# amzn/pecos

Measured on NVIDIA H100. Metric: XR-Linear top-10 queries/sec, higher is better.
Workload: dtype f32

## Files before the change

### include/pecos_b200.h

```cpp
#ifndef PECOS_B200_H_
#define PECOS_B200_H_

#include <stdbool.h>
#include <stddef.h>
#include <stdint.h>

#ifdef __cplusplus
extern "C" {
#endif

typedef struct {
    uint32_t rows, cols;
    uint64_t* col_ptr;
    uint32_t* row_idx;
    float* val;
} ScipyCscF32;

typedef struct {
    uint32_t rows, cols;
    uint64_t* row_ptr;
    uint32_t* col_idx;
    float* val;
} ScipyCsrF32;

// ... 166 lines not shown
void pb200_hnsw_launch_info(void* model_ptr, uint64_t* out);
void pb200_hnsw_get_info(void* model_ptr, uint64_t* out);
int pb200_hnsw_host_info(const char* model_dir, int metric, int sparse, uint64_t* out);
uint32_t pb200_hnsw_vcap_retries(void* model_ptr);



void pb200_sparse_block_distances(int device, int metric, const void* row_ptr, const void* ent, const void* q_ids, uint32_t nq,
                                  const void* col_ptr, const void* post, uint32_t c0, uint32_t nc, void* out, void* work,
                                  void* stream);
void pb200_sparse_candidate_distances(int device, int metric, const void* row_ptr, const void* ent, const void* cand, uint32_t n,
                                      uint32_t C, void* out, void* work, void* stream);

void* pb200_xlinear_host_load(const char* model_path, int kind);
void* pb200_xlinear_host_from_csc(const ScipyCscF32* W, const ScipyCscF32* C, float bias);
void* pb200_xlinear_host_prefix_layer(void* hptr);
void pb200_xlinear_host_free(void* hptr);
uint32_t pb200_xlinear_host_depth(void* hptr);
void pb200_xlinear_host_layer_dims(void* hptr, uint32_t layer, uint64_t* out);
void pb200_xlinear_host_layer_export(void* hptr, uint32_t layer, void* chunks32, uint32_t* meta, void* entries8,
                                     uint32_t* label_of_col);
int pb200_xlinear_host_plan_fits(void* hptr, uint32_t beam_size, uint32_t only_topk, uint32_t* out);
int pb200_xlinear_plan_fits(void* ptr, uint32_t beam_size, uint32_t only_topk, uint32_t* out);
uint32_t pb200_xlinear_plan_stride(void* ptr, int host, uint32_t beam_size, uint32_t only_topk);
uint32_t pb200_xlinear_beam_limit(int topk);

#ifdef __cplusplus
}
#endif
#endif
```

### pecos_b200/core.py

```python
import ctypes
import os
from ctypes import (
    CFUNCTYPE,
    POINTER,
    byref,
    c_bool,
    c_char_p,
    c_double,
    c_float,
    c_int,
    c_int32,
    c_size_t,
    c_uint32,
    c_uint64,
    c_void_p,
    cast,
)

import numpy as np
import scipy.sparse as smat

LIB_BASENAME = "libpecos_b200_float32.so"
LIB_DIR = os.path.join(os.path.dirname(os.path.abspath(__file__)), "lib")
LIB_PATH = os.path.join(LIB_DIR, LIB_BASENAME)
# ... 412 lines not shown
        fp(c.pb200_hnsw_get_counters, None, [c_void_p, POINTER(c_uint64)])
        fp(c.pb200_hnsw_set_stages, c_int, [c_void_p, c_int])
        fp(c.pb200_hnsw_launch_info, None, [c_void_p, POINTER(c_uint64)])
        fp(c.pb200_hnsw_get_info, None, [c_void_p, POINTER(c_uint64)])
        fp(c.pb200_hnsw_host_info, c_int, [c_char_p, c_int, c_int, POINTER(c_uint64)])
        fp(c.pb200_pairwise_ann_get_counters, None, [c_void_p, POINTER(c_uint64)])
        fp(c.pb200_pairwise_ann_kernel_ms, c_double, [c_void_p])
        fp(c.pb200_pairwise_ann_launch_info, None, [c_void_p, POINTER(c_uint64)])
        fp(c.pb200_pairwise_ann_dense_fits, c_int, [c_uint32, POINTER(c_uint32)])
        fp(c.pb200_pairwise_ann_host_info, c_int, [c_char_p, c_int, POINTER(c_uint64)])
        fp(c.pb200_sparse_block_distances, None, [c_int, c_int, c_void_p, c_void_p, c_void_p, c_uint32, c_void_p, c_void_p,
                                                  c_uint32, c_uint32, c_void_p, c_void_p, c_void_p])
        fp(c.pb200_sparse_candidate_distances, None, [c_int, c_int, c_void_p, c_void_p, c_void_p, c_uint32, c_uint32, c_void_p,
                                                      c_void_p, c_void_p])
        fp(c.pb200_xlinear_host_load, c_void_p, [c_char_p, c_int])
        fp(c.pb200_xlinear_host_prefix_layer, c_void_p, [c_void_p])
        fp(c.pb200_xlinear_host_free, None, [c_void_p])
        fp(c.pb200_xlinear_host_depth, c_uint32, [c_void_p])
        fp(c.pb200_xlinear_host_layer_dims, None, [c_void_p, c_uint32, POINTER(c_uint64)])
        fp(c.pb200_xlinear_host_layer_export, None, [c_void_p, c_uint32, c_void_p, c_void_p, c_void_p, c_void_p])
        fp(c.pb200_xlinear_host_plan_fits, c_int, [c_void_p, c_uint32, c_uint32, POINTER(c_uint32)])
        fp(c.pb200_xlinear_plan_fits, c_int, [c_void_p, c_uint32, c_uint32, POINTER(c_uint32)])
        fp(c.pb200_xlinear_plan_stride, c_uint32, [c_void_p, c_int, c_uint32, c_uint32])
        fp(c.pb200_xlinear_beam_limit, c_uint32, [c_int])
        fp(c.pb200_xlinear_cm_info, c_int, [c_void_p, c_int, POINTER(c_uint64)])

    def xlinear_check_layer_beam(self, b_prev):
        limit = int(self.clib_float32.pb200_xlinear_beam_limit(1))
        if b_prev > limit:
            raise ValueError(f"pecos_b200: the beam entering this layer would hold {b_prev} nodes, more than the supported "
                             f"maximum of {limit}")
# ... 30 lines not shown
        owner = _PinnedOwner(self, ptr, buf)
        arr = np.frombuffer(owner.buf, dtype=dtype, count=int(n))
        return _PinnedArray(arr, owner)

    def host_layer_layout_from_csc(self, W, C, bias):
        cw = ScipyCscF32.init_from(smat.csc_matrix(W, dtype=np.float32))
        cc = ScipyCscF32.init_from(smat.csc_matrix(C, dtype=np.float32))
        h = c_void_p(self.clib_float32.pb200_xlinear_host_from_csc(byref(cw), byref(cc), c_float(bias)))
        return self._export_host_model(h)

    def host_model_layout(self, model_path, is_mmap=False):
        c = self.clib_float32
        h = c_void_p(c.pb200_xlinear_host_load(model_path.encode("utf-8"), 1 if is_mmap else 0))
        return self._export_host_model(h)

    def host_prefix_layer_layout(self, model_path):
        c = self.clib_float32
        h = c_void_p(c.pb200_xlinear_host_load(model_path.encode("utf-8"), 0))
        try:
            m = c_void_p(c.pb200_xlinear_host_prefix_layer(h))
        finally:
            c.pb200_xlinear_host_free(h)
        return self._export_host_model(m)[0]

    def _export_host_model(self, h):
        c = self.clib_float32
        try:
            layers = []
            for d in range(c.pb200_xlinear_host_depth(h)):
                dims = (c_uint64 * 8)()
                c.pb200_xlinear_host_layer_dims(h, d, dims)
                w_rows, n_cols, out_cols, n_chunks, c_max, meta_len, n_ent, n_lab = [int(x) for x in dims]
                chunks = np.zeros(n_chunks, dtype=CHUNK_HEADER_DTYPE)
                meta = np.zeros(meta_len, dtype=np.uint32)
                entries = np.zeros(n_ent, dtype=CHUNK_ENTRY_DTYPE)
# ... 42 lines not shown
```

### pecos_b200/csrc/c_api.cu

```cuda
#include "../../include/pecos_b200.h"

#include <algorithm>
#include <atomic>
#include <cstdio>
#include <cstdlib>
#include <cstring>
#include <memory>
#include <exception>
#include <mutex>
#include <string>
#include <thread>
#include <unordered_set>
#include <vector>

#include "hnsw_build_sparse.h"
#include "hnsw_engine.h"
#include "pairwise_engine.h"
#include "xlinear_engine.h"

namespace {

std::atomic<int> g_device{0};

[[noreturn]] void die(const char* where, const char* what) {
// ... 693 lines not shown
    std::unique_ptr<pb200::XLinearHostModel> m =
        kind == 1 ? pb200::load_xlinear_mmap_model(model_path, false)
                  : pb200::load_xlinear_npz_model(model_path, pb200::LT_BINARY_SEARCH_CHUNKED);
    return m.release();
    PB200_API_END("pb200_xlinear_host_load")
}

void* pb200_xlinear_host_from_csc(const ScipyCscF32* W, const ScipyCscF32* C, float bias) {
    PB200_API_BEGIN
    const pb200::CscRaw w{W->rows, W->cols, W->col_ptr, W->row_idx, W->val};
    const pb200::CscRaw c{C->rows, C->cols, C->col_ptr, C->row_idx, C->val};
    return pb200::make_single_layer_model(w, c, bias).release();
    PB200_API_END("pb200_xlinear_host_from_csc")
}

void* pb200_xlinear_host_prefix_layer(void* hptr) {
    PB200_API_BEGIN
    const auto& H = *static_cast<pb200::XLinearHostModel*>(hptr);
    if (H.depth() < 2) throw std::runtime_error("pecos_b200: the prefix layer needs a model of depth >= 2");
    auto m = std::make_unique<pb200::XLinearHostModel>();
    m->layers.resize(1);
    pb200::build_prefix_layer(H.layers[0], H.layers[1], m->layers[0]);
    return m.release();
    PB200_API_END("pb200_xlinear_host_prefix_layer")
}

void pb200_xlinear_host_free(void* hptr) { delete static_cast<pb200::XLinearHostModel*>(hptr); }

int pb200_xlinear_host_plan_fits(void* hptr, uint32_t beam_size, uint32_t only_topk, uint32_t* out) {
    PB200_API_BEGIN
    if (!hptr) throw std::runtime_error("null host model");
    return plan_fits(*static_cast<pb200::XLinearHostModel*>(hptr), beam_size, only_topk, out);
    PB200_API_END("pb200_xlinear_host_plan_fits")
}

int pb200_xlinear_plan_fits(void* ptr, uint32_t beam_size, uint32_t only_topk, uint32_t* out) {
    PB200_API_BEGIN
    return plan_fits(xlinear_of(ptr).primary().host(), beam_size, only_topk, out);
    PB200_API_END("pb200_xlinear_plan_fits")
}
// ... 458 lines not shown
```

### pecos_b200/csrc/xlinear_cm_kernel.cuh

```cuda
#pragma once

constexpr int kCmFeat = 8;
constexpr int kCmSlots = 4;
constexpr int kCmMaxWarps = 16;
constexpr int kCmMinWarps = 4;
constexpr uint32_t kCmMaxDup = 400;
constexpr uint32_t kCmSmemBudget = 224u << 10;
constexpr uint32_t kCmMinReuse = 24;
constexpr uint32_t kCmMinPairsPerSm = 48u;
constexpr uint32_t kCmDirectRows = 16384;
constexpr uint32_t kCmEmpty = 0xFFFFFFFFu;

struct CmWork {
    uint32_t* slot_pos;
    uint32_t* count;
    uint32_t* bucket_ptr;
    uint64_t* cost_ptr;
    uint32_t* pair_q;
    uint32_t* pair_pos;
    uint32_t* claim;
    uint32_t* active;
};

struct CmPlan {
    bool eligible = false;
    uint32_t warps = 0, grid = 0;
    size_t smem = 0;
};

constexpr uint32_t kCmPrefixTop0 = 8;
struct CmPrefixOut {
    uint32_t rows = 0;
    uint32_t n0 = 0;
    int pp_kind = 0, pp_p = 0;
    const ChunkHeader* chunks1 = nullptr;
    uint32_t* beam_id = nullptr;
    float* beam_val = nullptr;
    uint32_t* beam_cnt = nullptr;
    uint32_t beam_stride = 0;
    float* cand1 = nullptr;
    uint64_t cand1_stride = 0;
};

__host__ __device__ inline uint32_t cm_align16(uint32_t x) { return (x + 15u) & ~15u; }

__host__ __device__ constexpr uint32_t cm_buffers(uint32_t stages) { return stages + 1u; }

__host__ __device__ inline size_t cm_warp_bytes(uint32_t acc_cols, uint32_t stages) {
// ... 332 lines not shown
}

__device__ inline uint32_t cm_start_chunk(const CmWork& w, uint32_t n_vc, uint32_t b, uint32_t shares) {
    const uint64_t T = w.cost_ptr[n_vc];
    if (T == 0) return n_vc;
    const uint64_t t = static_cast<uint64_t>(T / shares) * b + (T % shares) * b / shares;
    uint32_t lo = 0, hi = n_vc;
    while (hi - lo > 1) {
        const uint32_t mid = (lo + hi) >> 1;
        if (w.cost_ptr[mid] <= t) lo = mid; else hi = mid;
    }
    return lo;
}

enum { kCmPhSwitch, kCmPhCopy, kCmPhStaging, kCmPhLookup, kCmPhAccumulate, kCmPhSlice, kCmPhases };
#ifdef PB200_CM_TRACE
constexpr uint32_t kCmTraceCtas = 1024;
constexpr uint32_t kCmTraceWarp = kCmPhases + 4;
constexpr uint32_t kCmTraceCta = 3 + kCmMaxWarps * kCmTraceWarp;
__device__ unsigned long long g_cm_trace[3 + kCmTraceCtas * kCmTraceCta];
__device__ __forceinline__ unsigned long long cm_globaltimer() {
    unsigned long long t;
    asm volatile("mov.u64 %0, %%globaltimer;" : "=l"(t));
    return t;
}
struct CmTrace {
    unsigned long long start;
    long long t, ph[kCmPhases];
    unsigned long long trips, slots;
    unsigned long long slices, pairs, images;
// ... 62 lines not shown
    const unsigned short* __restrict__ rp_s = reinterpret_cast<const unsigned short*>(img + S.off_rp);
    const float* __restrict__ ew_s = reinterpret_cast<const float*>(img + S.off_ew);
    const unsigned char* __restrict__ ec_s = img + S.off_ec;
    const int lane = threadIdx.x & 31;
    const int warp = threadIdx.x >> 5;
    const int nwarps = blockDim.x >> 5;
    constexpr int kStride = kCmFeat + 1;
    constexpr int kBuf = 32 * kStride;
    constexpr int kNBuf = static_cast<int>(cm_buffers(STAGES));
    unsigned char* mine = smem_raw + S.img_bytes + static_cast<size_t>(warp) * cm_warp_bytes(S.acc_cols, STAGES);
    uint32_t* st_idx = reinterpret_cast<uint32_t*>(mine);
    float* st_val = reinterpret_cast<float*>(st_idx + kNBuf * kBuf);
    float* my_acc = st_val + kNBuf * kBuf + lane;

    __shared__ __align__(8) unsigned long long s_mbar;
    const uint32_t mbar = static_cast<uint32_t>(__cvta_generic_to_shared(&s_mbar));
    if (threadIdx.x == 0) {
        cm_mbar_init(mbar, 1u);
        asm volatile("fence.proxy.async.shared::cta;" ::: "memory");
    }
    __syncthreads();
    CmTrace trace;
    trace.begin();

    constexpr int kPerIter = 32 / kCmFeat;
    constexpr int kIters = 32 / kPerIter;
    const int sub = lane / kCmFeat, fl = lane % kCmFeat;
    uint32_t parity = 0;

    uint32_t e = 0, ee = 0, backlog = 0;
    float x = 0.0f;
    uint32_t hp = 0, l1_end = 0;
    auto add_rows = [&](uint32_t row, uint32_t cnt, uint32_t n_ent, bool drain) {
        const uint32_t l2_end = row + cnt;
// ... 41 lines not shown
        backlog = avail - added;
        trace.count(trips, added);
        l1_end = l2_end;
    };

    uint32_t bias_range = 0, n_cols = 0;
    auto stage_image = [&](uint32_t c) {
        if (threadIdx.x == 0) cm_bulk_load(static_cast<uint32_t>(__cvta_generic_to_shared(img)), images + static_cast<uint64_t>(c) * S.img_bytes, S.img_bytes, mbar);
        cm_mbar_wait(mbar, parity);
        parity ^= 1u;
        trace.staged();
        trace.mark(kCmPhCopy);
        bias_range = hdr_s[0];
        n_cols = hdr_s[1];
    };

    auto score_slice = [&](uint32_t s0, uint32_t s_end) {
        const uint32_t pidx = s0 + lane;
        const bool have = pidx < s_end;
        uint32_t q = 0, pos = 0, qn = 0;
        uint64_t qb = 0;
        if (have) {
            if constexpr (PREFIX) {
                q = pidx;
            } else {
                q = w.pair_q[pidx];
                pos = w.pair_pos[pidx];
            }
            qb = X.row_ptr[q] - X.nnz_base;
            qn = static_cast<uint32_t>(X.row_ptr[q + 1] - X.nnz_base - qb);
// ... 79 lines not shown
            trace.mark(kCmPhLookup);
            add_rows(static_cast<uint32_t>(buf * kBuf + lane * kStride), cnt, n_ent, false);
            trace.mark(kCmPhAccumulate);
            __syncwarp();
        }
        cm_cp_async_wait<0>();
        {
            const uint32_t o = static_cast<uint32_t>(buf * kBuf + lane * kStride);
            const uint32_t b0 = bias_range & 0xFFFFu, b1 = bias_range >> 16;
            const bool live = have && b1 > b0;
            st_idx[o] = bias_range;
            st_val[o] = L.bias;
            add_rows(o, live ? 1u : 0u, live ? b1 - b0 : 0u, true);
        }
        trace.mark(kCmPhAccumulate);
        if (have) {
            if constexpr (PREFIX) {
                unsigned long long key[kCmPrefixTop0];
#pragma unroll
                for (uint32_t j = 0; j < kCmPrefixTop0; ++j)
                    key[j] = j < P.n0 ? xl_exact_key(xl_transform(my_acc[j * 32], P.pp_kind, P.pp_p), j) : 0ull;
#pragma unroll
                for (uint32_t a = 1; a < kCmPrefixTop0; ++a)
#pragma unroll
                    for (uint32_t b = a; b > 0; --b)
                        if (key[b] > key[b - 1]) { const unsigned long long t = key[b]; key[b] = key[b - 1]; key[b - 1] = t; }
                const uint64_t o = static_cast<uint64_t>(q) * P.beam_stride;
                float* dst = P.cand1 + static_cast<uint64_t>(q) * P.cand1_stride;
#pragma unroll
                for (uint32_t r = 0; r < kCmPrefixTop0; ++r) {
                    if (r < P.n0) {
                        const uint32_t j = xl_exact_key_pos(key[r]);
                        P.beam_id[o + r] = j;
                        P.beam_val[o + r] = xl_exact_key_value(key[r]);
                        const ChunkHeader h = P.chunks1[j];
                        const float* src = my_acc + (P.n0 + h.col_begin) * 32u;
                        for (uint32_t col = 0; col < h.n_cols; ++col) dst[col] = src[col * 32];
                        dst += h.n_cols;
                    }
                }
                P.beam_cnt[q] = P.n0;
            }
        }
        if constexpr (!PREFIX) {
            float* tile = st_val + ((buf + kNBuf - 1) % kNBuf) * kBuf;
            const uint32_t n_pairs = s_end - s0;
            const uint64_t o_mine = have ? static_cast<uint64_t>(q) * cand_stride_q + pos : 0u;
            float* dst[kIters];
#pragma unroll
            for (int it = 0; it < kIters; ++it) dst[it] = cand + __shfl_sync(kFull, o_mine, it * kPerIter + sub) + fl;
            for (uint32_t c0 = 0; c0 < n_cols; c0 += kCmFeat) {
                const uint32_t nc = min(static_cast<uint32_t>(kCmFeat), n_cols - c0);
                __syncwarp();
#pragma unroll
                for (int k = 0; k < kCmFeat; ++k)
                    if (static_cast<uint32_t>(k) < nc) tile[lane * kStride + k] = my_acc[(c0 + k) * 32];
                __syncwarp();
                if (static_cast<uint32_t>(fl) < nc) {
#pragma unroll
                    for (int it = 0; it < kIters; ++it)
                        if (static_cast<uint32_t>(it * kPerIter + sub) < n_pairs) dst[it][c0] = tile[(it * kPerIter + sub) * kStride + fl];
                }
            }
        }
        trace.slice(s_end - s0);
        trace.mark(kCmPhSlice);
    };

    if constexpr (PREFIX) {
        const uint32_t begin = static_cast<uint32_t>(static_cast<uint64_t>(P.rows) * blockIdx.x / gridDim.x);
        const uint32_t end = static_cast<uint32_t>(static_cast<uint64_t>(P.rows) * (blockIdx.x + 1u) / gridDim.x);
        if (begin < end) {
            stage_image(0);
            for (uint32_t s0 = begin + static_cast<uint32_t>(warp) * 32u; s0 < end; s0 += static_cast<uint32_t>(nwarps) * 32u)
                score_slice(s0, min(s0 + 32u, end));
        }
        trace.flush(warp, lane, P.rows);
    } else {
        const uint32_t n_vc = S.n_vc;
        __shared__ unsigned long long s_pick_work[kCmMaxWarps];
        __shared__ uint32_t s_pick_act[kCmMaxWarps];
        __shared__ uint32_t s_pick_c[kCmMaxWarps];
        auto better = [n_vc](unsigned long long wa, uint32_t aa, uint32_t ca, unsigned long long wb, uint32_t ab, uint32_t cb) {
            if (ca == n_vc) return false;
            if (cb == n_vc) return true;
            const unsigned long long la = wa * (ab + 1u), lb = wb * (aa + 1u);
            return la > lb || (la == lb && ca < cb);
        };
        uint32_t c = cm_start_chunk(w, n_vc, blockIdx.x, gridDim.x);
        trace.mark(kCmPhSwitch);
        while (c < n_vc) {
            if (threadIdx.x == 0) atomicAdd(w.active + c, 1u);
// ... 22 lines not shown
            for (int d = 16; d > 0; d >>= 1) {
                const unsigned long long ow = __shfl_xor_sync(kFull, bw, d);
                const uint32_t oa = __shfl_xor_sync(kFull, ba, d);
                const uint32_t oc = __shfl_xor_sync(kFull, bc, d);
                if (better(ow, oa, oc, bw, ba, bc)) { bw = ow; ba = oa; bc = oc; }
            }
            if (lane == 0) { s_pick_work[warp] = bw; s_pick_act[warp] = ba; s_pick_c[warp] = bc; }
            __syncthreads();
            bw = s_pick_work[0];
            ba = s_pick_act[0];
            c = s_pick_c[0];
            for (int k = 1; k < nwarps; ++k)
                if (better(s_pick_work[k], s_pick_act[k], s_pick_c[k], bw, ba, c)) { bw = s_pick_work[k]; ba = s_pick_act[k]; c = s_pick_c[k]; }
            trace.mark(kCmPhSwitch);
        }
        trace.flush(warp, lane, w.bucket_ptr[n_vc]);
    }
}
```

### pecos_b200/csrc/xlinear_engine.cu

```cuda
#include "xlinear_engine.h"
#include "shard_merge.cuh"

#include <algorithm>
#include <atomic>
#include <cstring>
#include <exception>
#include <thread>

namespace pb200 {

namespace {

constexpr unsigned kFull = 0xFFFFFFFFu;
constexpr int kWarpsMax = 10;
constexpr int kMCap = 256;
constexpr int kMFlush = 128;
constexpr int kCSmem = 128;
constexpr int kQCap = 1024;
constexpr int kSortCap = 2048;
constexpr int kTopkThreads = 256;

constexpr int kMCapLookup = 256;

template <int MCAP>
// ... 929 lines not shown
                PB200_CUDA(cudaGetLastError());
                model_bytes_ += bytes;
            }
        }
        model_bytes_ += src.chunks.size() * sizeof(ChunkHeader) + src.meta.size() * 4 + src.entries.size() * 8 +
                        src.label_of_col.size() * 4;
    }
    if (layers_.size() >= 2 && layers_[0].view.featmap && layers_[1].view.featmap) {
        const ChunkedLayerHost& H0 = host_->layers[0];
        const ChunkedLayerHost& H1 = host_->layers[1];
        bool ok = H0.n_chunks == 1 && H0.n_cols >= 1 && H0.n_cols <= kCmPrefixTop0 && H1.n_chunks == H0.n_cols &&
                  !H0.reordered && !H1.reordered && H0.w_rows == H1.w_rows && H0.w_rows <= kCmDirectRows &&
                  std::memcmp(&H0.bias, &H1.bias, sizeof(float)) == 0 && H0.n_cols + H1.n_cols <= 256u;
        for (const ChunkHeader& ch : H0.chunks) ok = ok && !(ch.has_bias & kChunkAbsent);
        for (const ChunkHeader& ch : H1.chunks) ok = ok && !(ch.has_bias & kChunkAbsent);
        if (ok) {
            ChunkedLayerHost M;
            build_prefix_layer(H0, H1, M);
            const uint32_t fm_words = static_cast<uint32_t>((static_cast<uint64_t>(M.w_rows) + 31) / 32);
            const uint64_t n_ent = M.entries.size();
            CmShape shape = n_ent < 65535u ? cm_shape(fm_words, M.w_rows, M.r_max, static_cast<uint32_t>(n_ent), M.c_max, 1, 1) : CmShape{};
            if (shape.ok && shape.direct && shape.img_bytes <= cmimg_budget) {
                LayerStore& P = prefix_;
                P.chunks.upload(M.chunks.data(), M.chunks.size(), stream_);
                P.meta.upload(M.meta.data(), M.meta.size(), stream_);
                P.entries.upload(reinterpret_cast<const uint2*>(M.entries.data()), M.entries.size(), stream_);
                const uint32_t vc_ptr[2] = {0u, 1u};
                P.cm_vc_ptr.upload(vc_ptr, 2, stream_);
                P.view.chunks = P.chunks.get();
                P.view.meta = P.meta.get();
                P.view.entries = P.entries.get();
                P.view.n_cols = M.n_cols;
                P.view.n_chunks = 1;
                P.view.c_max = M.c_max;
                P.view.w_rows = M.w_rows;
                P.view.bias = M.bias;
                shape.vc_ptr = P.cm_vc_ptr.get();
                P.cm_shape = shape;
                P.cm_images.reserve(shape.img_bytes);
                xl_cm_build_images_kernel<<<1, 256, 0, stream_>>>(P.view, shape, P.cm_images.get());
                PB200_CUDA(cudaGetLastError());
                PB200_CUDA(cudaStreamSynchronize(stream_));
                model_bytes_ += shape.img_bytes + M.chunks.size() * sizeof(ChunkHeader) + M.meta.size() * 4 + M.entries.size() * 8 + 8;
            }
        }
    }
    PB200_CUDA(cudaStreamSynchronize(stream_));
    for (auto& l : host_->layers) {
        std::vector<uint32_t>().swap(l.meta);
        std::vector<ChunkEntry>().swap(l.entries);
    }
    const int max_smem = 200 * 1024;
    PB200_CUDA(cudaFuncSetAttribute(xl_chunk_scores_kernel<false, false, false>, cudaFuncAttributeMaxDynamicSharedMemorySize, max_smem));
    PB200_CUDA(cudaFuncSetAttribute(xl_chunk_scores_kernel<false, true, false>, cudaFuncAttributeMaxDynamicSharedMemorySize, max_smem));
    PB200_CUDA(cudaFuncSetAttribute(xl_chunk_scores_kernel<false, false, true>, cudaFuncAttributeMaxDynamicSharedMemorySize, max_smem));
    PB200_CUDA(cudaFuncSetAttribute(xl_chunk_scores_kernel<false, true, true>, cudaFuncAttributeMaxDynamicSharedMemorySize, max_smem));
    PB200_CUDA(cudaFuncSetAttribute(xl_chunk_scores_kernel<true, false, false>, cudaFuncAttributeMaxDynamicSharedMemorySize, max_smem));
    PB200_CUDA(cudaFuncSetAttribute(xl_chunk_scores_kernel<true, true, false>, cudaFuncAttributeMaxDynamicSharedMemorySize, max_smem));
    PB200_CUDA(cudaFuncSetAttribute(xl_topk_kernel, cudaFuncAttributeMaxDynamicSharedMemorySize, max_smem));
// ... 177 lines not shown
    } else {
        if (collect_stats) launch(xl_chunk_scores_kernel<false, true, false>);
        else launch(xl_chunk_scores_kernel<false, false, false>);
    }
    PB200_CUDA(cudaGetLastError());
    ++launches_;
    layer_profile_[d].scores_kernel = chunk_major ? 4 : query_warp ? 3 : dense ? 2 : lookup ? 1 : 0;
    return layer_profile_[d].scores_kernel;
}

bool XLinearEngine::use_prefix_(const QueryDev& q, const std::vector<LayerPlan>& plan) const {
    if (!prefix_.cm_shape.ok || !chunk_major_ || no_prefix_ || q.row_ptr == nullptr || !layers_[0].view.featmap || plan.size() < 2)
        return false;
    if (plan[0].k < host_->layers[0].n_cols) return false;
    if (static_cast<uint64_t>(q.rows) * std::max<uint32_t>(q.max_row_nnz, 1u) >= (1ull << 32)) return false;
    return cm_force_ || q.rows >= kCmMinPairsPerSm * n_sm_;
}

void XLinearEngine::launch_prefix_(const QueryDev& q, const std::vector<LayerPlan>& plan, uint32_t ws_row) {
    const CmShape& S = prefix_.cm_shape;
    const uint32_t rows = q.rows;
    const uint32_t grid = std::min<uint32_t>(n_sm_, (rows + 31u) / 32u);
    const uint32_t share = (rows + grid - 1) / grid;
    const uint32_t warps = std::max<uint32_t>(1u, std::min<uint32_t>(S.warps_fit, (share + 31u) / 32u));
    const size_t smem = S.img_bytes + warps * cm_warp_bytes(S.acc_cols, S.stages) + 64;
    CmPrefixOut P;
    P.rows = rows;
    P.n0 = host_->layers[0].n_cols;
    P.pp_kind = plan[0].pp.kind;
    P.pp_p = plan[0].pp.p;
    P.chunks1 = layers_[1].view.chunks;
    P.beam_id = bid_(1, ws_row);
    P.beam_val = bval_(1, ws_row);
    P.beam_cnt = bcnt_(1, ws_row);
    P.beam_stride = beam_stride_;
    P.cand1_stride = static_cast<uint64_t>(plan[1].b_prev) * std::max<uint32_t>(layers_[1].view.c_max, 1u);
    P.cand1 = cand_.get() + ws_row * P.cand1_stride;
    auto launch = [&](auto kernel) {
        kernel<<<grid, warps * 32, smem, stream_>>>(prefix_.view, q, CmWork{}, S, prefix_.cm_images.get(), nullptr, 0, P);
    };
    if (S.stages == 4) launch(xl_cm_scores_kernel<true, 4, true>);
    else launch(xl_cm_scores_kernel<true, 2, true>);
    PB200_CUDA(cudaGetLastError());
// ... 574 lines not shown
```

### pecos_b200/csrc/xlinear_engine.h

```cpp
#pragma once

#include <functional>
#include <memory>
#include <string>
#include <vector>

#include "cuda_util.h"
#include "xlinear_host.h"

namespace pb200 {

struct LayerDev {
    const ChunkHeader* chunks;
    const uint32_t* meta;
    const uint32_t* rowext;
    const uint2* entries;
    const uint32_t* label_of_col;
    const uint2* featmap;
    uint32_t fm_words;
    uint32_t n_cols;
    uint32_t n_chunks;
    uint32_t c_max;
    uint32_t w_rows;
    float bias;
// ... 84 lines not shown
    SelectedResult predict_selected(const HostMatrix& x, const HostMatrix& sel, const char* post_processor,
                                    const HostMatrix& codes = {});

    void resident_upload_csr(const HostMatrix& x);
    double resident_predict(uint32_t beam_size, const char* post_processor, uint32_t only_topk, bool collect_stats);
    Result resident_fetch();

    uint32_t sharded_local_csr_packed(const HostMatrix& x, uint32_t beam_size, const char* post_processor, uint32_t only_topk,
                                      uint32_t stride_capacity, void* rec_dev);
    Result sharded_merge_packed(uint32_t world, uint32_t rows, uint32_t stride, uint32_t only_topk, const void* g_rec);

    void set_profile(bool on) { profile_ = on; }
    void set_kernel_mode(int mode);
    bool has_feature_maps() const;
    const CmShape* cm_shape_of(int d) const {
        if (d < 0) return &prefix_.cm_shape;
        return static_cast<size_t>(d) < layers_.size() ? &layers_[d].cm_shape : nullptr;
    }
    const std::vector<XLinearLayerProfile>& layer_profile() const { return layer_profile_; }
    void reset_profile();
    const std::vector<XLinearStats>& layer_stats() const { return layer_stats_; }
    uint64_t launches() const { return launches_; }
    uint64_t model_bytes() const { return model_bytes_; }

private:
    struct LayerPlan {
        uint32_t k = 0;
        uint32_t b_prev = 0;
        uint32_t k_cap = 0;
        PostProc pp;
    };
    struct LayerStore {
// ... 80 lines not shown
    DeviceBuffer<uint32_t> shard_ids_, shard_cnt_;
    DeviceBuffer<float> shard_vals_;

    PinnedBuffer<uint32_t> out_ids_;
    PinnedBuffer<float> out_vals_;
    PinnedBuffer<uint32_t> out_cnt_;

    bool profile_ = false;
    bool no_query_warp_ = false;
    bool force_query_warp_ = false;
    bool no_topk_filter_ = false;
    bool chunk_major_ = true;
    bool cm_force_ = false;
    bool no_prefix_ = false;
    LayerStore prefix_;
    bool use_prefix_(const QueryDev& q, const std::vector<LayerPlan>& plan) const;
    void launch_prefix_(const QueryDev& q, const std::vector<LayerPlan>& plan, uint32_t ws_row);
    uint32_t n_sm_ = 132;
    DeviceBuffer<uint32_t> cm_slot_pos_, cm_count_, cm_claim_, cm_active_, cm_bucket_ptr_, cm_pair_q_, cm_pair_pos_;
    DeviceBuffer<uint64_t> cm_cost_ptr_;
    bool force_block_topk_ = false;
    std::vector<XLinearLayerProfile> layer_profile_;
    std::vector<XLinearStats> layer_stats_;
    uint64_t launches_ = 0;
    cudaEvent_t ev_[4] = {nullptr, nullptr, nullptr, nullptr};
};

}
```

### pecos_b200/csrc/xlinear_host.h

```cpp
#pragma once

#include <algorithm>
#include <cmath>
#include <thread>

#include "host_io.h"

namespace pb200 {

enum LayerTypeRequested { LT_CSC = 0, LT_HASH_CHUNKED = 1, LT_BINARY_SEARCH_CHUNKED = 2 };

enum PostProcKind { PP_NOOP = 0, PP_SIGMOID = 1, PP_LOG_SIGMOID = 2, PP_LP_HINGE = 3, PP_LOG_LP_HINGE = 4 };

struct PostProc {
    int kind = PP_NOOP;
    int p = 0;
};

inline PostProc parse_post_processor(const std::string& name) {
    auto starts = [&](const char* s) { size_t n = strlen(s); return name.size() >= n && name.compare(0, n, s) == 0; };
    auto ends = [&](const char* s) { size_t n = strlen(s); return name.size() >= n && name.compare(name.size() - n, n, s) == 0; };
    PostProc pp;
    if (name == "noop") return pp;
    if (name == "sigmoid") { pp.kind = PP_SIGMOID; return pp; }
// ... 278 lines not shown
            h.ent_off = entries.size();
            meta.insert(meta.end(), src_m, src_m + m_len);
            entries.insert(entries.end(), src_e, src_e + n_ent);
        } else {
            h.nnz_rows = 0;
            h.has_bias = kChunkAbsent;
            h.meta_off = 0;
            h.ent_off = 0;
        }
    }
    if (meta.empty()) meta.assign(4, 0u);
    L.meta.swap(meta);
    L.entries.swap(entries);
}

inline void build_prefix_layer(const ChunkedLayerHost& L0, const ChunkedLayerHost& L1, ChunkedLayerHost& M) {
    if (L0.reordered || L1.reordered || L0.w_rows != L1.w_rows) throw std::runtime_error("prefix layer: layers do not merge");
    CscHost W;
    W.rows = L0.w_rows;
    W.cols = L0.n_cols + L1.n_cols;
    W.col_ptr.assign(static_cast<size_t>(W.cols) + 1, 0);
    auto for_each_entry = [&](auto&& fn) {
        uint32_t first = 0;
        for (const ChunkedLayerHost* L : {&L0, &L1}) {
            for (const ChunkHeader& h : L->chunks) {
                const uint32_t* rows = L->meta.data() + h.meta_off;
                const uint32_t* rp = rows + round_up4(h.nnz_rows);
                const ChunkEntry* en = L->entries.data() + h.ent_off;
                for (uint32_t r = 0; r < h.nnz_rows; ++r)
                    for (uint32_t i = rp[r]; i < rp[r + 1]; ++i) fn(first + h.col_begin + en[i].col_offset, rows[r], en[i].val);
            }
            first += L->n_cols;
        }
    };
    for_each_entry([&](uint32_t col, uint32_t, float) { ++W.col_ptr[col + 1]; });
    for (uint32_t c = 0; c < W.cols; ++c) W.col_ptr[c + 1] += W.col_ptr[c];
    W.row_idx.resize(W.nnz());
    W.val.resize(W.nnz());
    std::vector<uint64_t> fill(W.col_ptr.begin(), W.col_ptr.end() - 1);
    for_each_entry([&](uint32_t col, uint32_t row, float v) {
        W.row_idx[fill[col]] = row;
        W.val[fill[col]++] = v;
    });
    build_chunked_layer(W, csc_ones_column(W.cols), L0.bias, M);
}

inline uint64_t feature_map_bytes(const ChunkedLayerHost& L) {
    return static_cast<uint64_t>(L.n_chunks) * ((static_cast<uint64_t>(L.w_rows) + 31) / 32) * 8;
}

inline void build_feature_map(ChunkedLayerHost& L) {
    L.fm_words = static_cast<uint32_t>((static_cast<uint64_t>(L.w_rows) + 31) / 32);
    L.featmap.assign(static_cast<uint64_t>(L.n_chunks) * L.fm_words, uint2_host{0u, 0u});
    parallel_for_chunks(L.n_chunks, [&](uint64_t p) {
        const ChunkHeader& h = L.chunks[p];
        const uint32_t* rows = L.meta.data() + h.meta_off;
        uint2_host* cells = L.featmap.data() + p * L.fm_words;
        for (uint32_t r = 0; r < h.nnz_rows; ++r) cells[rows[r] >> 5].x |= 1u << (rows[r] & 31u);
        uint32_t run = 0;
// ... 357 lines not shown
```

Measured before the change: 23.68 million.

## Split merged prefix layer into column groups across CTAs

The fused layer-0+layer-1 prefix layer is now split into up to two column groups. Each group carries all layer-0 columns plus a subset of layer-1 chunks in its own image, and CTAs are assigned per group. Each CTA scores only its group's columns and writes only the candidate columns whose top chunk falls in its group. This shrinks the per-CTA image and accumulator work and raises parallelism for small query batches. The cost is recomputing the layer-0 scores in every group, a larger image footprint, and a more complex write path driven by a bitmask.

```diff
diff --git a/include/pecos_b200.h b/include/pecos_b200.h
--- a/include/pecos_b200.h
+++ b/include/pecos_b200.h
@@ -204,7 +204,8 @@
 
 void* pb200_xlinear_host_load(const char* model_path, int kind);
 void* pb200_xlinear_host_from_csc(const ScipyCscF32* W, const ScipyCscF32* C, float bias);
-void* pb200_xlinear_host_prefix_layer(void* hptr);
+void* pb200_xlinear_host_prefix_layer(void* hptr, uint32_t groups);
+uint32_t pb200_xlinear_prefix_groups(uint32_t n0, uint32_t n_sm);
 void pb200_xlinear_host_free(void* hptr);
 uint32_t pb200_xlinear_host_depth(void* hptr);
 void pb200_xlinear_host_layer_dims(void* hptr, uint32_t layer, uint64_t* out);
diff --git a/pecos_b200/core.py b/pecos_b200/core.py
--- a/pecos_b200/core.py
+++ b/pecos_b200/core.py
@@ -450,7 +450,8 @@
         fp(c.pb200_sparse_candidate_distances, None, [c_int, c_int, c_void_p, c_void_p, c_void_p, c_uint32, c_uint32, c_void_p,
                                                       c_void_p, c_void_p])
         fp(c.pb200_xlinear_host_load, c_void_p, [c_char_p, c_int])
-        fp(c.pb200_xlinear_host_prefix_layer, c_void_p, [c_void_p])
+        fp(c.pb200_xlinear_host_prefix_layer, c_void_p, [c_void_p, c_uint32])
+        fp(c.pb200_xlinear_prefix_groups, c_uint32, [c_uint32, c_uint32])
         fp(c.pb200_xlinear_host_free, None, [c_void_p])
         fp(c.pb200_xlinear_host_depth, c_uint32, [c_void_p])
         fp(c.pb200_xlinear_host_layer_dims, None, [c_void_p, c_uint32, POINTER(c_uint64)])
@@ -511,11 +512,11 @@
         h = c_void_p(c.pb200_xlinear_host_load(model_path.encode("utf-8"), 1 if is_mmap else 0))
         return self._export_host_model(h)
 
-    def host_prefix_layer_layout(self, model_path):
+    def host_prefix_layer_layout(self, model_path, groups=1):
         c = self.clib_float32
         h = c_void_p(c.pb200_xlinear_host_load(model_path.encode("utf-8"), 0))
         try:
-            m = c_void_p(c.pb200_xlinear_host_prefix_layer(h))
+            m = c_void_p(c.pb200_xlinear_host_prefix_layer(h, groups))
         finally:
             c.pb200_xlinear_host_free(h)
         return self._export_host_model(m)[0]
diff --git a/pecos_b200/csrc/c_api.cu b/pecos_b200/csrc/c_api.cu
--- a/pecos_b200/csrc/c_api.cu
+++ b/pecos_b200/csrc/c_api.cu
@@ -731,16 +731,18 @@
     PB200_API_END("pb200_xlinear_host_from_csc")
 }
 
-void* pb200_xlinear_host_prefix_layer(void* hptr) {
+void* pb200_xlinear_host_prefix_layer(void* hptr, uint32_t groups) {
     PB200_API_BEGIN
     const auto& H = *static_cast<pb200::XLinearHostModel*>(hptr);
     if (H.depth() < 2) throw std::runtime_error("pecos_b200: the prefix layer needs a model of depth >= 2");
     auto m = std::make_unique<pb200::XLinearHostModel>();
     m->layers.resize(1);
-    pb200::build_prefix_layer(H.layers[0], H.layers[1], m->layers[0]);
+    pb200::build_prefix_layer(H.layers[0], H.layers[1], m->layers[0], groups);
     return m.release();
     PB200_API_END("pb200_xlinear_host_prefix_layer")
 }
+
+uint32_t pb200_xlinear_prefix_groups(uint32_t n0, uint32_t n_sm) { return pb200::prefix_groups_for(n0, n_sm); }
 
 void pb200_xlinear_host_free(void* hptr) { delete static_cast<pb200::XLinearHostModel*>(hptr); }
 
diff --git a/pecos_b200/csrc/xlinear_cm_kernel.cuh b/pecos_b200/csrc/xlinear_cm_kernel.cuh
--- a/pecos_b200/csrc/xlinear_cm_kernel.cuh
+++ b/pecos_b200/csrc/xlinear_cm_kernel.cuh
@@ -32,6 +32,8 @@
 struct CmPrefixOut {
     uint32_t rows = 0;
     uint32_t n0 = 0;
+    uint32_t n1 = 0;
+    uint32_t groups = 1;
     int pp_kind = 0, pp_p = 0;
     const ChunkHeader* chunks1 = nullptr;
     uint32_t* beam_id = nullptr;
@@ -394,6 +396,11 @@
 }
 
 enum { kCmPhSwitch, kCmPhCopy, kCmPhStaging, kCmPhLookup, kCmPhAccumulate, kCmPhSlice, kCmPhases };
+#ifdef PB200_CM_TRACE_PREFIX
+constexpr bool kCmTracePrefix = true;
+#else
+constexpr bool kCmTracePrefix = false;
+#endif
 #ifdef PB200_CM_TRACE
 constexpr uint32_t kCmTraceCtas = 1024;
 constexpr uint32_t kCmTraceWarp = kCmPhases + 4;
@@ -486,10 +493,17 @@
     float* my_acc = st_val + kNBuf * kBuf + lane;
 
     __shared__ __align__(8) unsigned long long s_mbar;
+    __shared__ uint32_t s_cb1[kCmPrefixTop0], s_w1[kCmPrefixTop0];
     const uint32_t mbar = static_cast<uint32_t>(__cvta_generic_to_shared(&s_mbar));
     if (threadIdx.x == 0) {
         cm_mbar_init(mbar, 1u);
         asm volatile("fence.proxy.async.shared::cta;" ::: "memory");
+    }
+    if constexpr (PREFIX) {
+        if (threadIdx.x < P.n0) {
+            s_cb1[threadIdx.x] = P.chunks1[threadIdx.x].col_begin;
+            s_w1[threadIdx.x] = P.chunks1[threadIdx.x].n_cols;
+        }
     }
     __syncthreads();
     CmTrace trace;
@@ -561,6 +575,8 @@
         bias_range = hdr_s[0];
         n_cols = hdr_s[1];
     };
+
+    uint32_t group = 0;
 
     auto score_slice = [&](uint32_t s0, uint32_t s_end) {
         const uint32_t pidx = s0 + lane;
@@ -670,8 +686,9 @@
             add_rows(o, live ? 1u : 0u, live ? b1 - b0 : 0u, true);
         }
         trace.mark(kCmPhAccumulate);
-        if (have) {
-            if constexpr (PREFIX) {
+        uint32_t ord = 0;
+        if constexpr (PREFIX) {
+            if (have) {
                 unsigned long long key[kCmPrefixTop0];
 #pragma unroll
                 for (uint32_t j = 0; j < kCmPrefixTop0; ++j)
@@ -682,40 +699,81 @@
                     for (uint32_t b = a; b > 0; --b)
                         if (key[b] > key[b - 1]) { const unsigned long long t = key[b]; key[b] = key[b - 1]; key[b - 1] = t; }
                 const uint64_t o = static_cast<uint64_t>(q) * P.beam_stride;
-                float* dst = P.cand1 + static_cast<uint64_t>(q) * P.cand1_stride;
 #pragma unroll
                 for (uint32_t r = 0; r < kCmPrefixTop0; ++r) {
                     if (r < P.n0) {
                         const uint32_t j = xl_exact_key_pos(key[r]);
-                        P.beam_id[o + r] = j;
-                        P.beam_val[o + r] = xl_exact_key_value(key[r]);
-                        const ChunkHeader h = P.chunks1[j];
-                        const float* src = my_acc + (P.n0 + h.col_begin) * 32u;
-                        for (uint32_t col = 0; col < h.n_cols; ++col) dst[col] = src[col * 32];
-                        dst += h.n_cols;
+                        ord |= j << (3u * r);
+                        if (group == 0) {
+                            P.beam_id[o + r] = j;
+                            P.beam_val[o + r] = xl_exact_key_value(key[r]);
+                        }
                     }
                 }
-                P.beam_cnt[q] = P.n0;
-            }
-        }
-        if constexpr (!PREFIX) {
+                if (group == 0) P.beam_cnt[q] = P.n0;
+            }
+        }
+        {
             float* tile = st_val + ((buf + kNBuf - 1) % kNBuf) * kBuf;
             const uint32_t n_pairs = s_end - s0;
-            const uint64_t o_mine = have ? static_cast<uint64_t>(q) * cand_stride_q + pos : 0u;
+            uint64_t o_mine = 0;
+            float* out = cand;
+            uint32_t n_out = n_cols;
+            uint32_t j_lo = 0, j_hi = 0, col_lo = 0, r = 0, j = 0, left = 0, src = 0;
+            if constexpr (PREFIX) {
+                out = P.cand1;
+                n_out = P.n1;
+                o_mine = have ? static_cast<uint64_t>(q) * P.cand1_stride : 0u;
+                j_lo = prefix_group_chunk(P.n0, P.groups, group);
+                j_hi = prefix_group_chunk(P.n0, P.groups, group + 1u);
+                col_lo = s_cb1[j_lo];
+                j = ord & 7u;
+                left = s_w1[j];
+                src = s_cb1[j];
+            } else {
+                o_mine = have ? static_cast<uint64_t>(q) * cand_stride_q + pos : 0u;
+            }
             float* dst[kIters];
 #pragma unroll
-            for (int it = 0; it < kIters; ++it) dst[it] = cand + __shfl_sync(kFull, o_mine, it * kPerIter + sub) + fl;
-            for (uint32_t c0 = 0; c0 < n_cols; c0 += kCmFeat) {
-                const uint32_t nc = min(static_cast<uint32_t>(kCmFeat), n_cols - c0);
+            for (int it = 0; it < kIters; ++it) dst[it] = out + __shfl_sync(kFull, o_mine, it * kPerIter + sub) + fl;
+            for (uint32_t c0 = 0; c0 < n_out; c0 += kCmFeat) {
+                const uint32_t nc = min(static_cast<uint32_t>(kCmFeat), n_out - c0);
+                uint32_t mask = 0;
                 __syncwarp();
 #pragma unroll
-                for (int k = 0; k < kCmFeat; ++k)
-                    if (static_cast<uint32_t>(k) < nc) tile[lane * kStride + k] = my_acc[(c0 + k) * 32];
+                for (int k = 0; k < kCmFeat; ++k) {
+                    if (static_cast<uint32_t>(k) < nc) {
+                        if constexpr (PREFIX) {
+                            if (have) {
+                                while (left == 0) {
+                                    ++r;
+                                    j = (ord >> (3u * r)) & 7u;
+                                    left = s_w1[j];
+                                    src = s_cb1[j];
+                                }
+                                if (j >= j_lo && j < j_hi) {
+                                    tile[lane * kStride + k] = my_acc[(P.n0 + src - col_lo) * 32];
+                                    mask |= 1u << k;
+                                }
+                                ++src;
+                                --left;
+                            }
+                        } else {
+                            tile[lane * kStride + k] = my_acc[(c0 + k) * 32];
+                        }
+                    }
+                }
                 __syncwarp();
+                uint32_t pm[kIters];
+#pragma unroll
+                for (int it = 0; it < kIters; ++it) {
+                    if constexpr (PREFIX) pm[it] = __shfl_sync(kFull, mask, it * kPerIter + sub);
+                    else pm[it] = static_cast<uint32_t>(it * kPerIter + sub) < n_pairs ? 0xFFu : 0u;
+                }
                 if (static_cast<uint32_t>(fl) < nc) {
 #pragma unroll
                     for (int it = 0; it < kIters; ++it)
-                        if (static_cast<uint32_t>(it * kPerIter + sub) < n_pairs) dst[it][c0] = tile[(it * kPerIter + sub) * kStride + fl];
+                        if ((pm[it] >> fl) & 1u) dst[it][c0] = tile[(it * kPerIter + sub) * kStride + fl];
                 }
             }
         }
@@ -724,14 +782,16 @@
     };
 
     if constexpr (PREFIX) {
-        const uint32_t begin = static_cast<uint32_t>(static_cast<uint64_t>(P.rows) * blockIdx.x / gridDim.x);
-        const uint32_t end = static_cast<uint32_t>(static_cast<uint64_t>(P.rows) * (blockIdx.x + 1u) / gridDim.x);
+        group = blockIdx.x % P.groups;
+        const uint32_t b = blockIdx.x / P.groups, ctas = gridDim.x / P.groups;
+        const uint32_t begin = static_cast<uint32_t>(static_cast<uint64_t>(P.rows) * b / ctas);
+        const uint32_t end = static_cast<uint32_t>(static_cast<uint64_t>(P.rows) * (b + 1u) / ctas);
         if (begin < end) {
-            stage_image(0);
+            stage_image(group);
             for (uint32_t s0 = begin + static_cast<uint32_t>(warp) * 32u; s0 < end; s0 += static_cast<uint32_t>(nwarps) * 32u)
                 score_slice(s0, min(s0 + 32u, end));
         }
-        trace.flush(warp, lane, P.rows);
+        if constexpr (kCmTracePrefix) trace.flush(warp, lane, P.rows * P.groups);
     } else {
         const uint32_t n_vc = S.n_vc;
         __shared__ unsigned long long s_pick_work[kCmMaxWarps];
@@ -784,6 +844,6 @@
                 if (better(s_pick_work[k], s_pick_act[k], s_pick_c[k], bw, ba, c)) { bw = s_pick_work[k]; ba = s_pick_act[k]; c = s_pick_c[k]; }
             trace.mark(kCmPhSwitch);
         }
-        trace.flush(warp, lane, w.bucket_ptr[n_vc]);
-    }
-}
+        if constexpr (!kCmTracePrefix) trace.flush(warp, lane, w.bucket_ptr[n_vc]);
+    }
+}
diff --git a/pecos_b200/csrc/xlinear_engine.cu b/pecos_b200/csrc/xlinear_engine.cu
--- a/pecos_b200/csrc/xlinear_engine.cu
+++ b/pecos_b200/csrc/xlinear_engine.cu
@@ -967,35 +967,59 @@
                   std::memcmp(&H0.bias, &H1.bias, sizeof(float)) == 0 && H0.n_cols + H1.n_cols <= 256u;
         for (const ChunkHeader& ch : H0.chunks) ok = ok && !(ch.has_bias & kChunkAbsent);
         for (const ChunkHeader& ch : H1.chunks) ok = ok && !(ch.has_bias & kChunkAbsent);
+        auto merged_shape = [](const ChunkedLayerHost& M) {
+            uint32_t e_max = 0;
+            for (const ChunkHeader& ch : M.chunks) {
+                const uint32_t* rp = M.meta.data() + ch.meta_off + round_up4(ch.nnz_rows);
+                e_max = std::max(e_max, rp[ch.nnz_rows]);
+            }
+            const uint32_t fm_words = static_cast<uint32_t>((static_cast<uint64_t>(M.w_rows) + 31) / 32);
+            return e_max < 65535u ? cm_shape(fm_words, M.w_rows, M.r_max, e_max, M.c_max, M.n_chunks, M.n_chunks) : CmShape{};
+        };
         if (ok) {
             ChunkedLayerHost M;
             build_prefix_layer(H0, H1, M);
-            const uint32_t fm_words = static_cast<uint32_t>((static_cast<uint64_t>(M.w_rows) + 31) / 32);
-            const uint64_t n_ent = M.entries.size();
-            CmShape shape = n_ent < 65535u ? cm_shape(fm_words, M.w_rows, M.r_max, static_cast<uint32_t>(n_ent), M.c_max, 1, 1) : CmShape{};
-            if (shape.ok && shape.direct && shape.img_bytes <= cmimg_budget) {
+            prefix_merged_shape_ = merged_shape(M);
+            ok = prefix_merged_shape_.ok && prefix_merged_shape_.direct;
+        }
+        if (ok) {
+            uint32_t groups = prefix_groups_for(H0.n_cols, n_sm_);
+            if (const char* env = std::getenv("PB200_PREFIX_GROUPS"))
+                groups = std::min<uint32_t>(std::max(std::atoi(env), 1), H0.n_cols);
+            ChunkedLayerHost M;
+            build_prefix_layer(H0, H1, M, groups);
+            CmShape shape = merged_shape(M);
+            const uint64_t bytes = static_cast<uint64_t>(shape.img_bytes) * groups;
+            if (shape.ok && shape.direct && bytes <= cmimg_budget) {
                 LayerStore& P = prefix_;
                 P.chunks.upload(M.chunks.data(), M.chunks.size(), stream_);
                 P.meta.upload(M.meta.data(), M.meta.size(), stream_);
                 P.entries.upload(reinterpret_cast<const uint2*>(M.entries.data()), M.entries.size(), stream_);
-                const uint32_t vc_ptr[2] = {0u, 1u};
-                P.cm_vc_ptr.upload(vc_ptr, 2, stream_);
+                std::vector<uint32_t> vc_ptr(groups + 1);
+                for (uint32_t g = 0; g <= groups; ++g) vc_ptr[g] = g;
+                P.cm_vc_ptr.upload(vc_ptr.data(), vc_ptr.size(), stream_);
                 P.view.chunks = P.chunks.get();
                 P.view.meta = P.meta.get();
                 P.view.entries = P.entries.get();
                 P.view.n_cols = M.n_cols;
-                P.view.n_chunks = 1;
+                P.view.n_chunks = groups;
                 P.view.c_max = M.c_max;
                 P.view.w_rows = M.w_rows;
                 P.view.bias = M.bias;
                 shape.vc_ptr = P.cm_vc_ptr.get();
                 P.cm_shape = shape;
-                P.cm_images.reserve(shape.img_bytes);
-                xl_cm_build_images_kernel<<<1, 256, 0, stream_>>>(P.view, shape, P.cm_images.get());
+                P.cm_images.reserve(bytes);
+                xl_cm_build_images_kernel<<<groups, 256, 0, stream_>>>(P.view, shape, P.cm_images.get());
                 PB200_CUDA(cudaGetLastError());
                 PB200_CUDA(cudaStreamSynchronize(stream_));
-                model_bytes_ += shape.img_bytes + M.chunks.size() * sizeof(ChunkHeader) + M.meta.size() * 4 + M.entries.size() * 8 + 8;
-            }
+                model_bytes_ += bytes + M.chunks.size() * sizeof(ChunkHeader) + M.meta.size() * 4 + M.entries.size() * 8 +
+                                vc_ptr.size() * 4;
+                prefix_groups_ = groups;
+            } else {
+                prefix_merged_shape_ = CmShape{};
+            }
+        } else {
+            prefix_merged_shape_ = CmShape{};
         }
     }
     PB200_CUDA(cudaStreamSynchronize(stream_));
@@ -1203,19 +1227,24 @@
         return false;
     if (plan[0].k < host_->layers[0].n_cols) return false;
     if (static_cast<uint64_t>(q.rows) * std::max<uint32_t>(q.max_row_nnz, 1u) >= (1ull << 32)) return false;
-    return cm_force_ || q.rows >= kCmMinPairsPerSm * n_sm_;
+    return cm_force_ || static_cast<uint64_t>(q.rows) * prefix_groups_ >= static_cast<uint64_t>(kCmMinPairsPerSm) * n_sm_;
 }
 
 void XLinearEngine::launch_prefix_(const QueryDev& q, const std::vector<LayerPlan>& plan, uint32_t ws_row) {
     const CmShape& S = prefix_.cm_shape;
     const uint32_t rows = q.rows;
-    const uint32_t grid = std::min<uint32_t>(n_sm_, (rows + 31u) / 32u);
-    const uint32_t share = (rows + grid - 1) / grid;
+    const uint32_t groups = prefix_groups_;
+    const uint32_t n0 = host_->layers[0].n_cols;
+    const uint32_t ctas = std::max<uint32_t>(1u, std::min<uint32_t>(n_sm_ / groups, (rows + 31u) / 32u));
+    const uint32_t grid = ctas * groups;
+    const uint32_t share = (rows + ctas - 1) / ctas;
     const uint32_t warps = std::max<uint32_t>(1u, std::min<uint32_t>(S.warps_fit, (share + 31u) / 32u));
     const size_t smem = S.img_bytes + warps * cm_warp_bytes(S.acc_cols, S.stages) + 64;
     CmPrefixOut P;
     P.rows = rows;
-    P.n0 = host_->layers[0].n_cols;
+    P.n0 = n0;
+    P.n1 = host_->layers[1].n_cols;
+    P.groups = groups;
     P.pp_kind = plan[0].pp.kind;
     P.pp_p = plan[0].pp.p;
     P.chunks1 = layers_[1].view.chunks;
diff --git a/pecos_b200/csrc/xlinear_engine.h b/pecos_b200/csrc/xlinear_engine.h
--- a/pecos_b200/csrc/xlinear_engine.h
+++ b/pecos_b200/csrc/xlinear_engine.h
@@ -122,8 +122,9 @@
     void set_kernel_mode(int mode);
     bool has_feature_maps() const;
     const CmShape* cm_shape_of(int d) const {
-        if (d < 0) return &prefix_.cm_shape;
-        return static_cast<size_t>(d) < layers_.size() ? &layers_[d].cm_shape : nullptr;
+        if (d == -1) return &prefix_merged_shape_;
+        if (d == -2) return &prefix_.cm_shape;
+        return d >= 0 && static_cast<size_t>(d) < layers_.size() ? &layers_[d].cm_shape : nullptr;
     }
     const std::vector<XLinearLayerProfile>& layer_profile() const { return layer_profile_; }
     void reset_profile();
@@ -234,6 +235,8 @@
     bool cm_force_ = false;
     bool no_prefix_ = false;
     LayerStore prefix_;
+    CmShape prefix_merged_shape_;
+    uint32_t prefix_groups_ = 1;
     bool use_prefix_(const QueryDev& q, const std::vector<LayerPlan>& plan) const;
     void launch_prefix_(const QueryDev& q, const std::vector<LayerPlan>& plan, uint32_t ws_row);
     uint32_t n_sm_ = 132;
diff --git a/pecos_b200/csrc/xlinear_host.h b/pecos_b200/csrc/xlinear_host.h
--- a/pecos_b200/csrc/xlinear_host.h
+++ b/pecos_b200/csrc/xlinear_host.h
@@ -316,23 +316,49 @@
     L.entries.swap(entries);
 }
 
-inline void build_prefix_layer(const ChunkedLayerHost& L0, const ChunkedLayerHost& L1, ChunkedLayerHost& M) {
+__host__ __device__ inline uint32_t prefix_group_chunk(uint32_t n0, uint32_t groups, uint32_t g) { return n0 * g / groups; }
+
+constexpr uint32_t kPrefixGroupsMax = 2;
+
+inline uint32_t prefix_groups_for(uint32_t n0, uint32_t n_sm) {
+    uint32_t g = std::max(1u, std::min(n0, kPrefixGroupsMax));
+    while (g > 1 && n_sm % g != 0) --g;
+    return g;
+}
+
+inline void build_prefix_layer(const ChunkedLayerHost& L0, const ChunkedLayerHost& L1, ChunkedLayerHost& M, uint32_t groups = 1) {
     if (L0.reordered || L1.reordered || L0.w_rows != L1.w_rows) throw std::runtime_error("prefix layer: layers do not merge");
+    const uint32_t n0 = L0.n_cols;
+    if (groups == 0 || (groups > 1 && (groups > n0 || L1.n_chunks != n0))) throw std::runtime_error("prefix layer: bad column groups");
     CscHost W;
     W.rows = L0.w_rows;
-    W.cols = L0.n_cols + L1.n_cols;
+    W.cols = groups * n0 + L1.n_cols;
     W.col_ptr.assign(static_cast<size_t>(W.cols) + 1, 0);
+    CscHost C;
+    C.rows = W.cols;
+    C.cols = groups;
+    C.col_ptr.assign(static_cast<size_t>(groups) + 1, 0);
+    C.row_idx.resize(W.cols);
+    C.val.assign(W.cols, 1.0f);
+    for (uint32_t i = 0; i < W.cols; ++i) C.row_idx[i] = i;
     auto for_each_entry = [&](auto&& fn) {
         uint32_t first = 0;
-        for (const ChunkedLayerHost* L : {&L0, &L1}) {
-            for (const ChunkHeader& h : L->chunks) {
-                const uint32_t* rows = L->meta.data() + h.meta_off;
+        for (uint32_t g = 0; g < groups; ++g) {
+            const uint32_t j_lo = prefix_group_chunk(n0, groups, g);
+            const uint32_t j_hi = g + 1 == groups ? L1.n_chunks : prefix_group_chunk(n0, groups, g + 1);
+            auto col_of = [&](uint32_t j) { return j < L1.n_chunks ? L1.chunks[j].col_begin : L1.n_cols; };
+            const uint32_t c_lo = col_of(j_lo);
+            auto chunk = [&](const ChunkedLayerHost& L, const ChunkHeader& h, uint32_t base) {
+                const uint32_t* rows = L.meta.data() + h.meta_off;
                 const uint32_t* rp = rows + round_up4(h.nnz_rows);
-                const ChunkEntry* en = L->entries.data() + h.ent_off;
+                const ChunkEntry* en = L.entries.data() + h.ent_off;
                 for (uint32_t r = 0; r < h.nnz_rows; ++r)
-                    for (uint32_t i = rp[r]; i < rp[r + 1]; ++i) fn(first + h.col_begin + en[i].col_offset, rows[r], en[i].val);
-            }
-            first += L->n_cols;
+                    for (uint32_t i = rp[r]; i < rp[r + 1]; ++i) fn(base + h.col_begin + en[i].col_offset, rows[r], en[i].val);
+            };
+            for (const ChunkHeader& h : L0.chunks) chunk(L0, h, first);
+            for (uint32_t j = j_lo; j < j_hi; ++j) chunk(L1, L1.chunks[j], first + n0 - c_lo);
+            first += n0 + col_of(j_hi) - c_lo;
+            C.col_ptr[g + 1] = first;
         }
     };
     for_each_entry([&](uint32_t col, uint32_t, float) { ++W.col_ptr[col + 1]; });
@@ -344,7 +370,7 @@
         W.row_idx[fill[col]] = row;
         W.val[fill[col]++] = v;
     });
-    build_chunked_layer(W, csc_ones_column(W.cols), L0.bias, M);
+    build_chunked_layer(W, C, L0.bias, M);
 }
 
 inline uint64_t feature_map_bytes(const ChunkedLayerHost& L) {
```

Result: no change. 23.84 million, median of 6 (+0.7%).
